# HKUST-Aerial-Robotics/Omni-swarm

Measured on AMD Instinct MI355X. Metric: keyframes/sec (4x fisheye 600x480) + p50 loop-match ms @ 100k-frame DB, higher is better.
Workload: dtype f16

## Files before the change

### include/omni_hip.h

```cpp
#ifndef OMNI_HIP_H
#define OMNI_HIP_H

#include <stddef.h>
#include <stdint.h>

#ifdef __cplusplus
extern "C" {
#endif

#define OMNI_ABI_VERSION 2

enum {
    OMNI_OK = 0,
    OMNI_ERR_INVALID = 1,
    OMNI_ERR_HIP = 2,
    OMNI_ERR_NOMEM = 3,
    OMNI_ERR_CAPACITY = 4
};

enum { OMNI_PREC_F32 = 0,
       OMNI_PREC_F16 = 1,
       OMNI_PREC_SPLIT = 2 };

enum { OMNI_STORE_F32 = 0, OMNI_STORE_F16 = 1 };
// ... 53 lines not shown

static inline void omni_fisheye_mask_rows(int height, int fisheye_mask, int* row0, int* row1) {
    *row0 = fisheye_mask ? height * 3 / 4 : height;
    *row1 = fisheye_mask ? height * 3 / 4 + height / 4 : height;
}

int omni_sp_infer(omni_sp* sp, const uint8_t* gray_host, int stride, int batch, int fisheye_mask,
                  float* kps_xy, int* n_kps, float* desc, float* scores);
int omni_sp_enqueue_dev(omni_sp* sp, const uint8_t* gray_dev, int stride, int batch, int fisheye_mask);
int omni_sp_fetch(omni_sp* sp, int batch, float* kps_xy, int* n_kps, float* desc, float* scores);
int omni_sp_dev_outputs(omni_sp* sp, const float** kps_xy_dev, const int** n_kps_dev, const float** desc_dev,
                        const float** scores_dev);
int omni_sp_get_dense(omni_sp* sp, int batch, float* semi_host, float* desc_host);
int omni_sp_postprocess_dense(omni_sp* sp, const float* semi_host, const float* desc_host, int batch,
                              float* kps_xy, int* n_kps, float* desc, float* scores);
int omni_sp_debug_layer(omni_sp* sp, const char* name, int batch, float* out_nchw_host, int* C, int* H, int* W);
#define OMNI_SP_NUM_STAGES 16
int         omni_sp_profile(omni_sp* sp, const uint8_t* gray_dev, int stride, int batch, int reps, float* stage_ms);
int         omni_sp_set_perf(omni_sp* sp, int on);
int         omni_sp_last_stage_ms(omni_sp* sp, float* stage_ms);
const char* omni_sp_stage_name(int stage);
double      omni_sp_stage_flops(const omni_sp* sp, int stage);
double      omni_sp_stage_tiles_left_out(const omni_sp* sp, int stage);
int         omni_sp_mask_skip_plan(int width, int height, int precision, int layer, int* rect, double* frac);

enum { OMNI_VLAD_CONV3X3_RELU6 = 0, OMNI_VLAD_PW_RELU6 = 1, OMNI_VLAD_DW3X3_RELU6 = 2,
       OMNI_VLAD_PW_LINEAR = 3, OMNI_VLAD_PW_LINEAR_RES = 4 };
typedef struct omni_vlad_layer {
    int kind, cin, cout, stride;
    const float* weight;
    const float* bias;
} omni_vlad_layer;
typedef struct omni_vlad_weights {
    int n_layers;
    const omni_vlad_layer* layers;
    int n_clusters, feat_dim, out_dim;
    const float* assign_w;
    const float* assign_b;
    const float* clusters;
    const float* fc_w;
    const float* fc_b;
} omni_vlad_weights;

omni_vlad* omni_vlad_create(omni_ctx* ctx, const omni_vlad_weights* w, int width, int height, int max_batch);
void       omni_vlad_destroy(omni_vlad* v);
int        omni_vlad_set_precision(omni_vlad* v, int precision);
// ... 169 lines not shown
```

### omni-swarm_amd/capi.py

```python
from __future__ import annotations

import ctypes as C
import os

import numpy as np

_HERE = os.path.dirname(os.path.abspath(__file__))
LIB_PATH = os.environ.get("OMNI_LIB") or os.path.join(_HERE, "lib", "libomni_hip.so")

OK, ERR_INVALID, ERR_HIP, ERR_NOMEM, ERR_CAPACITY = 0, 1, 2, 3, 4
PREC_F32, PREC_F16, PREC_SPLIT = 0, 1, 2
STORE_F32, STORE_F16 = 0, 1
BF_OPENCV, BF_MUTUAL = 0, 1
ABI_VERSION = 2
SP_NUM_LAYERS = 12
SP_NUM_STAGES = 16
SP_LAYER_NAMES = ["conv1a", "conv1b", "conv2a", "conv2b", "conv3a", "conv3b", "conv4a", "conv4b",
                  "convPa", "convPb", "convDa", "convDb"]
VB_NAMES = ["hblock", "sblock", "mblock", "pw_mfma3", "valu"]
VLAD_STEM_NAMES = ["stem", "stem_b0", "layers"]
VLAD_KINDS = {"conv3x3": 0, "pw_relu6": 1, "dw3x3_relu6": 2, "pw_linear": 3, "pw_linear_res": 4}

SYMBOLS = [
    "omni_abi_version", "omni_last_error", "omni_ctx_create", "omni_ctx_create_priority", "omni_ctx_order_after", "omni_memcpy_d2h_async", "omni_ctx_destroy", "omni_ctx_sync", "omni_ctx_stream",
    "omni_ctx_device_info", "omni_ctx_mfma_ceiling", "omni_dev_alloc", "omni_dev_free", "omni_host_alloc", "omni_host_free", "omni_memcpy_h2d", "omni_memcpy_d2h", "omni_timer_start",
    "omni_timer_stop", "omni_sp_create", "omni_sp_destroy", "omni_sp_desc_dim", "omni_sp_image_size", "omni_sp_infer", "omni_sp_enqueue_dev",
    "omni_sp_fetch", "omni_sp_dev_outputs", "omni_sp_get_dense", "omni_sp_postprocess_dense", "omni_sp_debug_layer",
    "omni_sp_profile", "omni_sp_stage_name", "omni_sp_stage_flops", "omni_sp_stage_tiles_left_out", "omni_sp_mask_skip_plan", "omni_vlad_create", "omni_vlad_destroy", "omni_vlad_set_precision", "omni_vlad_pack_block", "omni_sp_pack_constants",
    "omni_vlad_infer", "omni_vlad_enqueue_dev", "omni_vlad_fetch", "omni_vlad_dev_output", "omni_vlad_mask_skip_layers", "omni_vlad_debug_taps", "omni_vlad_debug_layer", "omni_vlad_block_paths", "omni_index_create",
    "omni_index_destroy", "omni_index_add", "omni_index_add_dev", "omni_index_ntotal", "omni_index_dim", "omni_index_reset", "omni_index_truncate", "omni_index_cert_stats",
    "omni_index_search", "omni_index_search_dev", "omni_index_search_prefix_dev", "omni_index_search_batch_prefix_dev", "omni_index_set_shard", "omni_topk_merge", "omni_index_last_scan_ms",
    "omni_index_save", "omni_index_load",
    "omni_trace_push", "omni_trace_pop", "omni_sp_set_perf", "omni_sp_last_stage_ms", "omni_bf_match", "omni_bf_match_multi", "omni_bf_match_batched_dev", "omni_config_count", "omni_config_describe", "omni_config_value", "omni_config_is_process_wide", "omni_cam_create", "omni_cam_create_mono", "omni_cam_destroy", "omni_cam_enqueue_dev", "omni_cam_enqueue_host", "omni_cam_enqueue_host_parts", "omni_cam_enqueue_fisheye_dev", "omni_cam_enqueue_fisheye_host", "omni_cam_get_input", "omni_cam_wait", "omni_cam_order_after", "omni_cam_set_active", "omni_cam_ready",
    "omni_shard_unique_id", "omni_shard_library_path", "omni_shard_create", "omni_shard_destroy", "omni_shard_ntotal", "omni_shard_preload_local", "omni_shard_step_batch_dev", "omni_shard_step_enqueue", "omni_shard_rows_consumed", "omni_shard_step_wait", "omni_shard_last_exchange_us",
    "omni_shard_search", "omni_flatten_create", "omni_flatten_destroy", "omni_flatten_out_bytes", "omni_flatten_enqueue_dev",
    "omni_resize_create", "omni_resize_destroy", "omni_resize_mode", "omni_resize_enqueue_dev", "omni_cam_enqueue_raw_dev", "omni_cam_enqueue_raw_host", "omni_cam_enqueue_raw_host_parts",
    "omni_landmarks_enqueue_dev", "omni_cam_set_stereo_model", "omni_cam_set_poses", "omni_cam_landmarks",
    "omni_homography_ransac_multi", "omni_bf_match_homography_multi", "omni_pnp_ransac_multi",
    "omni_jpeg_create", "omni_jpeg_destroy", "omni_jpeg_enqueue_dev", "omni_jpeg_header", "omni_jpeg_encode_host", "omni_cam_set_jpeg", "omni_cam_jpeg",
]
JPEG_OK, JPEG_TRUNCATED, JPEG_HEADER_BYTES = 0, 1, 328
HG_UNFILTERED, HG_OK, HG_NO_MODEL, HG_HOST = 0, 1, 2, 3
PNP_SKIPPED, PNP_OK, PNP_NO_MODEL, PNP_HOST = 0, 1, 2, 3
PNP_MAX_POINTS, PNP_MAX_ITERS = 2048, 1000


class OmniError(RuntimeError):
    pass


class _SpWeights(C.Structure):
# ... 84 lines not shown
    sig("omni_dev_free", C.c_int, [_vp, _vp])
    sig("omni_host_alloc", _vp, [C.c_size_t])
    sig("omni_host_free", C.c_int, [_vp])
    sig("omni_memcpy_h2d", C.c_int, [_vp, _vp, _vp, C.c_size_t])
    sig("omni_memcpy_d2h", C.c_int, [_vp, _vp, _vp, C.c_size_t])
    sig("omni_timer_start", C.c_int, [_vp])
    sig("omni_timer_stop", C.c_int, [_vp, _fp])
    sig("omni_sp_create", _vp, [_vp, C.POINTER(_SpWeights), _fp, _fp, C.c_int, C.c_int, C.c_int, C.c_float, C.c_int,
                                C.c_int, C.c_int])
    sig("omni_sp_destroy", None, [_vp])
    sig("omni_sp_desc_dim", C.c_int, [_vp])
    sig("omni_sp_infer", C.c_int, [_vp, _vp, C.c_int, C.c_int, C.c_int, _fp, _ip, _fp, _fp])
    sig("omni_sp_enqueue_dev", C.c_int, [_vp, _vp, C.c_int, C.c_int, C.c_int])
    sig("omni_sp_fetch", C.c_int, [_vp, C.c_int, _fp, _ip, _fp, _fp])
    sig("omni_sp_dev_outputs", C.c_int, [_vp, C.POINTER(_vp), C.POINTER(_vp), C.POINTER(_vp), C.POINTER(_vp)])
    sig("omni_sp_get_dense", C.c_int, [_vp, C.c_int, _fp, _fp])
    sig("omni_sp_postprocess_dense", C.c_int, [_vp, _fp, _fp, C.c_int, _fp, _ip, _fp, _fp])
    sig("omni_sp_debug_layer", C.c_int, [_vp, C.c_char_p, C.c_int, _fp, _ip, _ip, _ip])
    sig("omni_sp_profile", C.c_int, [_vp, _vp, C.c_int, C.c_int, C.c_int, _fp])
    sig("omni_sp_stage_name", C.c_char_p, [C.c_int])
    sig("omni_sp_stage_flops", C.c_double, [_vp, C.c_int])
    sig("omni_sp_stage_tiles_left_out", C.c_double, [_vp, C.c_int])
    sig("omni_sp_mask_skip_plan", C.c_int, [C.c_int, C.c_int, C.c_int, C.c_int, C.POINTER(C.c_int), C.POINTER(C.c_double)])
    sig("omni_vlad_create", _vp, [_vp, C.POINTER(_VladWeights), C.c_int, C.c_int, C.c_int])
    sig("omni_vlad_destroy", None, [_vp])
    sig("omni_vlad_set_precision", C.c_int, [_vp, C.c_int])
    sig("omni_sp_pack_constants", C.c_int64, [C.c_int, _fp, _fp, C.c_int, _vp, C.c_int64, C.POINTER(C.c_float)])
    sig("omni_vlad_pack_block", C.c_int64, [C.c_int, C.c_int, C.c_int, C.c_int, _fp, _fp, _fp, _fp, _fp, _vp, C.c_int64])
    sig("omni_vlad_infer", C.c_int, [_vp, _vp, C.c_int, C.c_int, C.c_int, _fp])
    sig("omni_vlad_enqueue_dev", C.c_int, [_vp, _vp, C.c_int, C.c_int, C.c_int])
    sig("omni_vlad_fetch", C.c_int, [_vp, C.c_int, _fp])
    sig("omni_vlad_dev_output", C.c_int, [_vp, C.POINTER(_vp)])
    sig("omni_vlad_mask_skip_layers", C.c_int, [_vp, C.POINTER(C.c_double), C.c_int])
    sig("omni_vlad_debug_taps", C.c_int, [_vp, C.c_int])
    sig("omni_vlad_debug_layer", C.c_int, [_vp, C.c_char_p, C.c_int, _fp, _ip, _ip, _ip])
    sig("omni_vlad_block_paths", C.c_int, [_vp, _ip, C.c_int])
    sig("omni_index_create", _vp, [_vp, C.c_int, C.c_int, C.c_int64])
    sig("omni_index_destroy", None, [_vp])
    sig("omni_index_add", C.c_int, [_vp, C.c_int64, _fp])
    sig("omni_index_add_dev", C.c_int, [_vp, C.c_int64, _vp])
    sig("omni_index_ntotal", C.c_int64, [_vp])
    sig("omni_index_reset", C.c_int, [_vp])
    sig("omni_index_truncate", C.c_int, [_vp, C.c_int64])
    sig("omni_index_cert_stats", C.c_int, [_vp, _i64p, _i64p])
    sig("omni_index_dim", C.c_int, [_vp])
    sig("omni_sp_image_size", C.c_int, [_vp, C.POINTER(C.c_int), C.POINTER(C.c_int)])
# ... 633 lines not shown
        src = self.ctx.to_device(g)
        out = self.ctx.to_device(np.full(n * self.capacity + guard, 0xA5, np.uint8))
        meta = self.ctx.to_device(np.full(2 * n, -1, np.int32))
        try:
            self.enqueue_dev(src, st, n, self.h_img if zero_from_row < 0 else zero_from_row, out, meta, meta + 4 * n)
            raw = self.ctx.from_device(out, (n * self.capacity + guard,), np.uint8)
            m = self.ctx.from_device(meta, (2, n), np.int32)
        finally:
            for p in (src, out, meta):
                self.ctx.free(p)
        self.last_raw = raw[:n * self.capacity].reshape(n, self.capacity)
        self.last_guard_ok = bool((raw[n * self.capacity:] == 0xA5).all())
        self.last_sizes = m[0].copy()
        return [(int(m[1, i]), self.last_raw[i, :m[0, i]].tobytes()) for i in range(n)]
SHARD_ID_BYTES = 128


def shard_unique_id() -> bytes:
    buf = C.create_string_buffer(SHARD_ID_BYTES)
    _check(lib().omni_shard_unique_id(buf))
    return buf.raw


def sp_mask_skip_plan(width: int, height: int, precision: int, layer: int):
    rect = (C.c_int * 4)()
    frac = C.c_double()
    _check(lib().omni_sp_mask_skip_plan(width, height, precision, layer, rect, C.byref(frac)))
    return tuple(rect), frac.value


def config_table() -> list:
    out = []
    for i in range(lib().omni_config_count()):
        env, doc = C.c_char_p(), C.c_char_p()
        d, lo, hi, cls = C.c_int(), C.c_int(), C.c_int(), C.c_int()
        _check(lib().omni_config_describe(i, C.byref(env), C.byref(d), C.byref(lo), C.byref(hi), C.byref(cls), C.byref(doc)))
        out.append({"env": env.value.decode(), "default": d.value, "lo": lo.value, "hi": hi.value, "cls": cls.value, "doc": doc.value.decode()})
    return out


def config_value(env: str) -> int:
    v = C.c_int()
    _check(lib().omni_config_value(env.encode(), C.byref(v)))
    return v.value


# ... 291 lines not shown
```

### omni-swarm_amd/csrc/config.h

```cpp
#pragma once
#include "common.h"

namespace omni {

enum CfgId {
    CFG_CONV_V1 = 0, CFG_RS_TRN, CFG_DET16, CFG_SP_SPARSE_DESC, CFG_SP_SPARSE_DA, CFG_SP_FUSED_CAND, CFG_SP_SPLIT_DB, CFG_SP_MASK_SKIP, CFG_SP_MASK_SKIP_SPLIT, CFG_SPLIT_FUSE1A, CFG_SPLIT_WINO,
    CFG_SPLIT_TRN, CFG_CONV_XCD, CFG_SP_PROFILE_MASK, CFG_PP_U8, CFG_PP_TRACE, CFG_PP_DBG, CFG_RS_TRACE, CFG_SPLIT_TRACE, CFG_SPLIT_DBG, CFG_WINO_TRACE, CFG_ROCTX,
    CFG_VLAD_BIG, CFG_VLAD_STEM_FUSE, CFG_VLAD_UNFUSED, CFG_VLAD_MFMA, CFG_VLAD_SBLOCK, CFG_VLAD_MBLOCK_PX, CFG_VLAD_MFMA_PX, CFG_VLAD_FC_MFMA, CFG_VLAD_MBLOCK_CPW,
    CFG_VLAD_SB_LDSPAD, CFG_VLAD_SB_PERSIST, CFG_VLAD_SB_TRACE, CFG_VLAD_SB_DBG, CFG_VLAD_MASK_SKIP,
    CFG_SCAN_ROWS_MIN, CFG_MQ_ROT, CFG_MQ_MIN, CFG_INDEX_MIRROR, CFG_INDEX_MIRROR_MIN_ROWS, CFG_INDEX_CERT_FAIL,
    CFG_GEOMETRY_THREADS, CFG_MESSAGE_THREADS, CFG_GEOMETRY_ASYNC, CFG_DETECTOR_ASYNC, CFG_PIPELINE_ONE_STREAM, CFG_PIPELINE_FIFO, CFG_PIPELINE_UNIT_PLAN,
    CFG_HW_QUEUES,
    CFG_RCCL_LIB,
    CFG_COUNT
};
enum CfgClass {
    CFG_VARIANT = 0,
    CFG_TUNING = 1,
    CFG_DEBUG = 2,
    CFG_TEST = 3,
    CFG_STRING = 4
};
struct CfgOption { const char* env; int def, lo, hi; int cls; const char* doc; };
extern const CfgOption kCfgOptions[CFG_COUNT];

struct Config {
    int v[CFG_COUNT];
    int operator[](CfgId i) const { return v[i]; }
};
// ... 6 lines not shown
```

### omni-swarm_amd/csrc/config.hip

```cpp
#include "config.h"

#include <atomic>
#include <cerrno>
#include <climits>
#include <cstdlib>

namespace omni {

const CfgOption kCfgOptions[CFG_COUNT] = {
    {"OMNI_CONV_V1", 0, 0, 3, CFG_VARIANT, "fp16 3x3 layers: 0 = production (conv1a fused into the ping-pong conv1b, register-stationary cin=128); 1 = generic kernel, 2 = persistent LDS-DMA kernel, "
                                           "3 = ping-pong without the conv1a fusion -- 1-3 exist only in the test build of the library (lib_test/)"},
    {"OMNI_RS_TRN", -1, -1, 1, CFG_VARIANT, "register-stationary kernel of the unpooled cin=128 fp16 layers: tile orientation, -1 = the one with fewer tiles, 0 = plain, 1 = transposed"},
    {"OMNI_DET16", 1, 0, 1, CFG_VARIANT, "detector head of the fp16 and OMNI_PREC_SPLIT paths on v_mfma_f32_32x32x16_f16 with split (hi, lo) operands (0: the exact-f32 MFMA kernel)"},
    {"OMNI_SP_SPARSE_DESC", 1, 0, 1, CFG_VARIANT, "convDb + descriptor norm only at the cells around the key points (0: dense descriptor map)"},
    {"OMNI_SP_SPARSE_DA", 1, 0, 1, CFG_VARIANT, "convDa only at those cells too (fp16 and OMNI_PREC_SPLIT; 0: dense convDa)"},
    {"OMNI_SP_FUSED_CAND", 1, 0, 1, CFG_VARIANT, "getKeyPoints' threshold inside the detector head's epilogue + window masks from the candidate list (0: sp_cand_kernel re-reads the heat map)"},
    {"OMNI_SP_SPLIT_DB", 1, 0, 1, CFG_VARIANT, "OMNI_PREC_SPLIT: convDb + descriptor norm at the key points' cells with split (hi, lo) operands on the fp16 matrix cores (0: exact-f32 MFMA convolution)"},
    {"OMNI_SP_MASK_SKIP", 1, 0, 1, CFG_VARIANT, "fp16: the tiles inside the constant region of the fisheye mask are left out of the tile walk (0: every tile)"},
    {"OMNI_SP_MASK_SKIP_SPLIT", 1, 0, 1, CFG_VARIANT, "the same for OMNI_PREC_SPLIT"},
    {"OMNI_SPLIT_FUSE1A", 1, 0, 1, CFG_VARIANT, "OMNI_PREC_SPLIT: conv1a built inside the conv1b kernel from the u8 image (0: separate exact-f32 conv1a pass)"},
    {"OMNI_SPLIT_WINO", 7, 0, 15, CFG_VARIANT, "OMNI_PREC_SPLIT: the cin = 64 layers as Winograd F(2x2,3x3) kernels with split operands (conv_wino.hip), bit 0 = conv1b (with the conv1a "
                                                "fusion), 1 = conv2a, 2 = conv2b, 3 = conv3a (off by default: same time as the direct kernel, profiles/r06g); 0: the direct kernels of conv_split.hip"},
    {"OMNI_SPLIT_TRN", -1, -1, 1, CFG_VARIANT, "OMNI_PREC_SPLIT cin=128 kernel: tile orientation, as OMNI_RS_TRN"},
    {"OMNI_CONV_XCD", 1, 0, 1, CFG_VARIANT, "persistent convolution kernels derive (cout group, tile walk) from an XCD-aware block id: the cout groups of a pixel tile and its neighbours "
                                           "share one L2 (0: plain blockIdx; process-wide, same results either way)"},
    {"OMNI_SP_PROFILE_MASK", 0, 0, 1, CFG_TUNING, "omni_sp_profile times the stages with the fisheye mask on (what the key-frame pipeline runs)"},
    {"OMNI_PP_U8", 1, 0, 1, CFG_VARIANT, "fp16 conv1a inside conv1b's kernel: matrix-core operands straight from the image bytes (0: through the 256-entry u8 -> (hi, lo) table in LDS)"},
    {"OMNI_PP_TRACE", 0, 0, 1, CFG_DEBUG, "s_memtime trace of the ping-pong conv kernel on stderr"},
    {"OMNI_PP_DBG", 0, 0, 255, CFG_DEBUG, "ping-pong conv kernel timing ablations (WRONG results)"},
    {"OMNI_RS_TRACE", 0, 0, 1, CFG_DEBUG, "s_memtime trace of the register-stationary kernel"},
    {"OMNI_SPLIT_TRACE", 0, 0, 1, CFG_DEBUG, "s_memtime trace of the split-precision kernel"},
    {"OMNI_SPLIT_DBG", 0, 0, 3, CFG_DEBUG, "split-precision kernel timing ablations: 1 = no stores, 2 = every DMA reads tile 0 (WRONG results)"},
    {"OMNI_WINO_TRACE", 0, 0, 1, CFG_DEBUG, "s_memtime trace of the Winograd split kernel"},
    {"OMNI_ROCTX", 0, 0, 1, CFG_DEBUG, "roctx ranges around upload / SuperPoint / MobileNetVLAD / post-processing / BF match / index add + search / exchange and the host loop's "
                                      "stages (rocprofv3 --marker-trace; the library is resolved by dlopen)"},
    {"OMNI_VLAD_BIG", 0, 0, 128, CFG_TUNING, "64 / 128: the 64- / 128-pixel tiles of the unfused block kernel (measured slower at 600x480)"},
    {"OMNI_VLAD_STEM_FUSE", 1, 0, 1, CFG_VARIANT, "stem + block 0 in one kernel (0: two kernels)"},
    {"OMNI_VLAD_UNFUSED", 0, 0, 1, CFG_VARIANT, "1: every block as expand / depthwise / project launches"},
    {"OMNI_VLAD_MFMA", 1, 0, 1, CFG_VARIANT, "late blocks' 1x1 convolutions on the matrix cores"},
    {"OMNI_VLAD_SBLOCK", 1, 0, 1, CFG_VARIANT, "fused split-fp16 block kernel (vlad_s.hip)"},
    {"OMNI_VLAD_MBLOCK_PX", 2048, 0, 1 << 24, CFG_TUNING, "fused matrix-core block kernel for blocks of at most this many input pixels per image (0 disables)"},
    {"OMNI_VLAD_MFMA_PX", 0, 0, 1 << 24, CFG_TUNING, "> 0: matrix-core 1x1 convolutions for blocks of at most this many input pixels per image (default 2048)"},
// ... 122 lines not shown
```

### omni-swarm_amd/csrc/conv.h

```cpp
#pragma once
#include "common.h"
#include "tile_walk.h"

namespace omni {

#define CONV_TH 8
#define CONV_TW 32
#define RS_TH 6
#define RS_TW 32
int conv_rs_pool_tile_rows();
#define CONV_COUT_TILE 64
#define CONV_CIN_CHUNK 64

static inline size_t conv_packed_elems(int cin, int cout, int ksize) { return (size_t)cin * cout * ksize * ksize; }

void conv_pack_weights_f16(const float* w_oihw, int cin, int cout, int ksize, __half* out);
void conv_pack_weights_f32(const float* w_oihw, int cin, int cout, int ksize, float* out);

struct ConvArgs {
    const void* in;
    void* out;
    const void* w_packed;
    const float* bias;
    int batch, H, W, cin, cout, ksize;
    int in_cstride = 0;
    bool relu, pool;
    bool out_f32;
    int n_cu = 0;
    const void* zero_page = nullptr;
    float split_inv = 0.f;
    int variant = 0;
    int skip_ty0 = 0, skip_ty1 = 0, skip_tx0 = 0, skip_tx1 = 0;
};
int conv_mfma(hipStream_t stream, int precision, const ConvArgs& a);
int conv_read_pixel_f16(hipStream_t stream, const void* map, int Ho, int Wo, int C, int y, int x, void* vec);
int conv_fill_rect_f16(hipStream_t stream, void* map, int batch, int Ho, int Wo, int C, int y0, int y1, int x0, int x1, const void* vec);
int conv_read_pixel_bytes(hipStream_t stream, const void* map, int64_t row_bytes, int64_t org_bytes, int pix_bytes, int y, int x, void* vec);
int conv_fill_rect_bytes(hipStream_t stream, void* map, int batch, int64_t img_bytes, int64_t row_bytes, int64_t org_bytes, int pix_bytes, int y0, int y1, int x0, int x1,
                         const void* vec);

float conv_pack_weights_split(const float* w_oihw, int cin, int cout, uint16_t* out);
float conv_split_act_scale();
int conv_split(hipStream_t stream, const ConvArgs& a);
int conv1a_split(hipStream_t stream, const uint8_t* gray, int stride, int batch, int H, int W, int fisheye_mask, const float* w, const float* bias,
                 const float* u8_lut, void* out_split, int skip_tr0 = 0, int skip_tr1 = 0);
int split_to_nchw_f32(hipStream_t stream, const void* in_split, float* out, int batch, int C, int H, int W);
void conv1a_split_pack_fused(const float* w , const float* bias , uint16_t* frag );
int conv1ab_split_fused(hipStream_t stream, const ConvArgs& a, const uint8_t* gray, int gstride, int fisheye_mask, const void* w1a_frag, const uint32_t* lut_hl);
float conv_pack_weights_wino(const float* w_oihw, int cin, int cout, uint16_t* out);
int conv_wino(hipStream_t stream, const ConvArgs& a, bool out_split);
int conv1ab_wino_fused(hipStream_t stream, const ConvArgs& a, const uint8_t* gray, int gstride, int fisheye_mask, const void* w1a_frag, const uint32_t* lut_hl, bool out_split);
int split_to_raw32(hipStream_t stream, const void* in_split, void* out_raw, int batch, int C, int H, int W);
int conv_read_pixels2x2_bytes(hipStream_t stream, const void* map, int64_t row_bytes, int64_t org_bytes, int pix_bytes, int y, int x, void* vec);
int conv_fill_rect2x2_bytes(hipStream_t stream, void* map, int batch, int64_t img_bytes, int64_t row_bytes, int64_t org_bytes, int pix_bytes, int y0, int y1, int x0, int x1,
                            const void* vec);
int raw32_to_nchw_f32(hipStream_t stream, const void* in_raw, float* out, int batch, int C, int H, int W);
__host__ __device__ inline int split_frame_w(int W) { return ((W + 31) & ~31) + 2; }
__host__ __device__ inline int split_frame_h(int H) { return ((H + 31) & ~31) + 2; }
inline size_t split_frame_bytes(int H, int W, int C) { return (size_t)split_frame_h(H) * split_frame_w(W) * C * 4; }

int conv1ab_fused(hipStream_t stream, const ConvArgs& a, const uint8_t* gray, int gstride, int fisheye_mask, const _Float16* w1a_frag,
                  const float* bias1a, const uint32_t* lut_hl);
// ... 46 lines not shown
```

### omni-swarm_amd/csrc/conv.hip

```cpp
#include "config.h"
#include "conv.h"
#include <type_traits>

namespace omni {

typedef _Float16 half8_t __attribute__((ext_vector_type(8)));
typedef _Float16 half4_t __attribute__((ext_vector_type(4)));
typedef float floatx16 __attribute__((ext_vector_type(16)));
typedef float floatx4 __attribute__((ext_vector_type(4)));

template <typename T, int KG, int EPL>
static void pack_weights(const float* w, int cin, int cout, int ks, T* out) {
    const int taps = ks * ks, n_ct = cout / 64, n_ch = cin / 64;
    size_t o = 0;
    for (int ct = 0; ct < n_ct; ++ct)
        for (int ch = 0; ch < n_ch; ++ch)
            for (int tap = 0; tap < taps; ++tap)
                for (int kg = 0; kg < KG; ++kg)
                    for (int m = 0; m < 2; ++m)
                        for (int l = 0; l < 64; ++l)
                            for (int e = 0; e < EPL; ++e) {
                                const int co = ct * 64 + m * 32 + (l & 31);
                                const int ci = ch * 64 + kg * (64 / KG) + (l >> 5) * EPL + e;
                                const float v = w[((size_t)co * cin + ci) * taps + tap];
// ... 2343 lines not shown
    const int y = (int)(by % rh);
    const int64_t b = by / rh;
    *reinterpret_cast<uint4*>(map + b * img_bytes + org_bytes + (y0 + y) * row_bytes + ((int64_t)(x0 + x) * chunks + c) * 16) = vec[c];
}
int conv_read_pixel_bytes(hipStream_t st, const void* map, int64_t row_bytes, int64_t org_bytes, int pix_bytes, int y, int x, void* vec) {
    OMNI_REQUIRE(pix_bytes % 16 == 0 && y >= 0 && x >= 0 && (org_bytes + y * row_bytes + (int64_t)x * pix_bytes) % 16 == 0, OMNI_ERR_INVALID, "conv_read_pixel_bytes: bad pixel");
    const int chunks = pix_bytes / 16;
    hipLaunchKernelGGL(read_pixel_f16_kernel, dim3(cdiv(chunks, 64)), dim3(64), 0, st, (const uint4*)map, (org_bytes + y * row_bytes + (int64_t)x * pix_bytes) / 16, chunks, (uint4*)vec);
    OMNI_LAUNCH_CHECK();
    return OMNI_OK;
}
int conv_fill_rect_bytes(hipStream_t st, void* map, int batch, int64_t img_bytes, int64_t row_bytes, int64_t org_bytes, int pix_bytes, int y0, int y1, int x0, int x1,
                         const void* vec) {
    OMNI_REQUIRE(pix_bytes % 16 == 0 && img_bytes % 16 == 0 && row_bytes % 16 == 0 && org_bytes % 16 == 0 && y0 >= 0 && x0 >= 0, OMNI_ERR_INVALID, "conv_fill_rect_bytes: bad layout");
    if (y1 <= y0 || x1 <= x0 || batch <= 0) return OMNI_OK;
    const int chunks = pix_bytes / 16;
    const int64_t total = (int64_t)batch * (y1 - y0) * (x1 - x0) * chunks;
    hipLaunchKernelGGL(fill_rect_bytes_kernel, dim3((unsigned)cdiv64(total, 256)), dim3(256), 0, st, (char*)map, img_bytes, row_bytes, org_bytes, chunks, y0, x0, y1 - y0,
                       x1 - x0, (const uint4*)vec, total);
    OMNI_LAUNCH_CHECK();
    return OMNI_OK;
}

}
```

### omni-swarm_amd/csrc/superpoint.hip

```cpp
#include <algorithm>
#include <vector>

#include "config.h"
#include "conv.h"
#include "sp_plan.h"
#include "sp_post.h"

namespace {
struct LayerDef { const char* name; int cin, cout, ks, div; bool pool; };
const LayerDef kLayers[OMNI_SP_NUM_LAYERS] = {
    {"conv1a", 1, 64, 3, 1, false},    {"conv1b", 64, 64, 3, 1, true},     {"conv2a", 64, 64, 3, 2, false},    {"conv2b", 64, 64, 3, 2, true},
    {"conv3a", 64, 128, 3, 4, false},  {"conv3b", 128, 128, 3, 4, true},   {"conv4a", 128, 128, 3, 8, false},  {"conv4b", 128, 128, 3, 8, false},
    {"convPa", 128, 256, 3, 8, false}, {"convPb", 256, 65, 1, 8, false},   {"convDa", 128, 256, 3, 8, false},  {"convDb", 256, 256, 1, 8, false}};
enum { L1A = 0, L1B, L2A, L2B, L3A, L3B, L4A, L4B, LPA, LPB, LDA, LDB };
enum { ST_CONV1A = 0, ST_CONV1B, ST_CONV2A, ST_CONV2B, ST_CONV3A, ST_CONV3B, ST_CONV4A, ST_CONV4B, ST_HEADS_A,
       ST_DET_TAIL, ST_DESC_TAIL, ST_POST, ST_COUNT };
const char* kStageNames[OMNI_SP_NUM_STAGES] = {
    "conv1a", "conv1b+pool", "conv2a", "conv2b+pool", "conv3a", "conv3b+pool", "conv4a", "conv4b", "convPa|convDa",
    "convPb+softmax+d2s", "convDb+l2norm", "nms+topk+describe", "", "", "", ""};
}

struct omni_sp {
    omni_ctx* ctx = nullptr;
    omni::Config cfg;
// ... 20 lines not shown
    void* wDbFragHi = nullptr; void* wDbFragLo = nullptr;
    float* bias_heads = nullptr;
    float* lut = nullptr;
    uint16_t* w1a_frag = nullptr;
    uint32_t* lut_hl = nullptr;
    void* wpk_w[OMNI_SP_NUM_LAYERS] = {};
    float winv_w[OMNI_SP_NUM_LAYERS] = {};
    void* a_tmp = nullptr;
    float* pca_compT = nullptr;
    float* pca_mean = nullptr;
    void *a1a = nullptr, *a1b = nullptr, *a2a = nullptr, *a2b = nullptr, *a3a = nullptr, *a3b = nullptr, *a4a = nullptr,
         *a4b = nullptr, *heads = nullptr;
    float *draw = nullptr, *semi = nullptr;
    uint8_t* gray_stage = nullptr;
    omni::SpPostBuffers pb = {};
    omni::HostBuf hstage;
    omni::DevBuf dense_tmp;
    hipEvent_t ev[OMNI_SP_NUM_STAGES + 1] = {};
    hipEvent_t ev_convs = nullptr;
    bool perf = false, perf_valid = false;
    struct MaskSkip {
        int ty0 = 0, ty1 = 0, tx0 = 0, tx1 = 0;
        int oy0 = 0, oy1 = 0, ox0 = 0, ox1 = 0;
        int oh = 0, ow = 0, oc = 0;
        int pix_bytes = 0;
        int64_t row_bytes = 0, img_bytes = 0, org_bytes = 0;
        void* vec = nullptr;
        void** map = nullptr;
        double frac = 0.0;
    };
    MaskSkip mskip[6];
    uint8_t* zero_gray = nullptr;
    size_t zero_gray_bytes = 0;
    std::mutex mu;
};

namespace omni {

template <typename T>
static int dev_upload(omni_sp* s, T** dst, const void* src, size_t bytes) {
    hipStream_t st = s->ctx->stream;
    if (int rc = s->mem.alloc(dst, bytes)) return rc;
    OMNI_HIP_TRY(hipMemcpyAsync(*dst, src, bytes, hipMemcpyHostToDevice, st));
    OMNI_HIP_TRY(hipStreamSynchronize(st));
    return OMNI_OK;
}

static void sp_mask_skip_rects(int H, int W, bool split, omni_sp::MaskSkip (&ks)[6]) {
    int m0, m1;
    omni_fisheye_mask_rows(H, 1, &m0, &m1);
    int h = H, w = W;
    for (auto& k : ks) k = omni_sp::MaskSkip{};
    int a = m0 + 1, b = (m1 == h) ? h - 1 : m1 - 2, c = 0, d = w - 1;
    if (split && b >= a) {
        omni_sp::MaskSkip& k = ks[0];
        k.ty0 = (a + 7) / 8; k.ty1 = (b + 1) / 8; k.tx0 = 0; k.tx1 = (w + 31) / 32;
        if (k.ty1 <= k.ty0) k.ty0 = k.ty1 = k.tx0 = k.tx1 = 0;
        k.oy0 = k.ty0 * 8; k.oy1 = k.ty1 * 8 < h ? k.ty1 * 8 : h; k.ox0 = 0; k.ox1 = k.ty1 > k.ty0 ? w : 0;
        k.oh = h; k.ow = w; k.oc = 64;
        k.frac = (double)(k.ty1 - k.ty0) / ((h + 7) / 8);
    }
    const bool pool[5] = {true, false, true, false, true};
    const int chans[5] = {64, 64, 64, 128, 128};
    static_assert(CONV_TW == 32, "tile width");
    const int TW = 32;
    for (int i = 0; i < 5; ++i) {
        const int TH = split ? (i == 4 ? 2 : 4) : (i == 4 ? conv_rs_pool_tile_rows() : CONV_TH);
        a += 1; b -= 1; c += 1; d -= 1;
        omni_sp::MaskSkip& k = ks[1 + i];
        if (b < a || d < c) break;
        k.ty0 = (a + TH - 1) / TH; k.ty1 = (b + 1) / TH; k.tx0 = (c + TW - 1) / TW; k.tx1 = (d + 1) / TW;
        if (k.ty1 <= k.ty0 || k.tx1 <= k.tx0) k.ty0 = k.ty1 = k.tx0 = k.tx1 = 0;
        k.frac = (double)(k.ty1 - k.ty0) * (k.tx1 - k.tx0) / ((double)((h + TH - 1) / TH) * ((w + TW - 1) / TW));
        const int f = pool[i] ? 2 : 1;
        k.oy0 = k.ty0 * TH / f; k.oy1 = k.ty1 * TH / f; k.ox0 = k.tx0 * TW / f; k.ox1 = k.tx1 * TW / f;
        if (pool[i]) { a = (a + 1) / 2; b = (b - 1) >> 1; c = (c + 1) / 2; d = (d - 1) >> 1; h /= 2; w /= 2; }
        k.oh = h; k.ow = w; k.oc = chans[i];
    }
}

static int sp_plan_mask_skip(omni_sp* s) {
    s->facts.mask_skip = false;
    const bool split = s->precision == OMNI_PREC_SPLIT;
    if (s->facts.conv_variant != 0 || s->precision == OMNI_PREC_F32) return OMNI_OK;
    if (!s->cfg[split ? CFG_SP_MASK_SKIP_SPLIT : CFG_SP_MASK_SKIP]) return OMNI_OK;
    sp_mask_skip_rects(s->H, s->W, split, s->mskip);
    void** maps[6] = {&s->a1a, &s->a1b, &s->a2a, &s->a2b, &s->a3a, &s->a3b};
    for (int i = 0; i < 6; ++i) {
        omni_sp::MaskSkip& k = s->mskip[i];
        k.map = maps[i];
        if (k.oc == 0) continue;
        if (split) {
            k.pix_bytes = k.oc * 4;
            k.row_bytes = (int64_t)split_frame_w(k.ow) * k.pix_bytes;
            k.img_bytes = (int64_t)split_frame_bytes(k.oh, k.ow, k.oc);
            k.org_bytes = k.row_bytes + k.pix_bytes;
        } else {
            k.pix_bytes = k.oc * 2; k.row_bytes = (int64_t)k.ow * k.pix_bytes; k.img_bytes = k.row_bytes * k.oh; k.org_bytes = 0;
        }
        if (k.ty1 > k.ty0) {
            if (int rc = s->mem.alloc(&k.vec, (size_t)k.pix_bytes * 4)) return rc;
            s->facts.mask_skip = true;
        }
    }
    return OMNI_OK;
}

static void sp_set_facts(omni_sp* s) {
    SpHandleFacts& f = s->facts;
    f.precision = s->precision; f.H = s->H; f.W = s->W;
    f.conv_variant = s->cfg[CFG_CONV_V1];
    f.det16 = s->cfg[CFG_DET16] != 0;
    f.fused_cand = s->cfg[CFG_SP_FUSED_CAND] != 0;
    f.sparse_desc = s->cfg[CFG_SP_SPARSE_DESC] != 0;
    f.sparse_da = s->cfg[CFG_SP_SPARSE_DA] != 0;
    f.split_fuse1a = s->cfg[CFG_SPLIT_FUSE1A] != 0;
    f.split_db = s->cfg[CFG_SP_SPLIT_DB] != 0;
    f.wino = sp_wino_layers(s->precision, s->cfg[CFG_SPLIT_WINO], s->H, s->W, f.split_fuse1a);
}

static int sp_init(omni_sp* s, const omni_sp_weights* w, const float* pca_comp, const float* pca_mean) {
    hipStream_t st = s->ctx->stream;
    int rc;
// ... 136 lines not shown
    s->pb.pca_mean = s->pca_mean;
    for (int i = 0; i <= OMNI_SP_NUM_STAGES; ++i) OMNI_HIP_TRY(hipEventCreate(&s->ev[i]));
    OMNI_HIP_TRY(hipEventCreateWithFlags(&s->ev_convs, hipEventDisableTiming));
    OMNI_HIP_TRY(hipStreamSynchronize(st));
    return sp_plan_mask_skip(s);
}

static int tails_prec(const SpPassPlan& p) { return p.tails_f32 ? OMNI_PREC_F32 : OMNI_PREC_F16; }

enum SpKernelFamily { SP_K_DIRECT, SP_K_WINO };
static ConvArgs sp_layer_args(const omni_sp* s, const SpPassPlan& p, int l, SpKernelFamily fam, const void* in, void* out, int batch, int cout = 0) {
    const LayerDef& d = kLayers[l];
    const bool split = s->precision == OMNI_PREC_SPLIT, wino = fam == SP_K_WINO;
    ConvArgs a;
    a.in = in; a.out = out; a.batch = batch; a.H = s->H / d.div; a.W = s->W / d.div; a.cin = d.cin; a.cout = cout ? cout : d.cout; a.ksize = d.ks;
    a.relu = l != LDB; a.pool = d.pool;
    a.out_f32 = l == LDB || (l == LPA && split);
    if (l == LDB) a.in_cstride = 512;
    a.w_packed = wino ? s->wpk_w[l] : s->wpk[l];
    a.split_inv = wino ? s->winv_w[l] : s->winv[l];
    a.bias = l == LPA ? s->bias_heads : (split && !a.out_f32) ? s->bias_s[l] : s->bias[l];
    a.n_cu = s->ctx->prop.multiProcessorCount; a.zero_page = s->ctx->zero_page; a.variant = s->facts.conv_variant;
    const int i = l == L1B ? 1 : l == L2A ? 2 : l == L2B ? 3 : l == L3A ? 4 : l == L3B ? 5 : -1;
    if (p.use_skip && i >= 0) { a.skip_ty0 = s->mskip[i].ty0; a.skip_ty1 = s->mskip[i].ty1; a.skip_tx0 = s->mskip[i].tx0; a.skip_tx1 = s->mskip[i].tx1; }
    return a;
}
static int sp_conv(omni_sp* s, const SpPassPlan& p, int l, const void* in, void* out, int batch, int cout = 0) {
    const ConvArgs a = sp_layer_args(s, p, l, SP_K_DIRECT, in, out, batch, cout);
    if (l == LDB) return conv_mfma(s->ctx->stream, tails_prec(p), a);
    return s->precision == OMNI_PREC_SPLIT ? conv_split(s->ctx->stream, a) : conv_mfma(s->ctx->stream, s->precision, a);
}
static int sp_heads_layer(omni_sp* s, const SpPassPlan& p, int batch, bool cpa_only) {
    return sp_conv(s, p, LPA, s->a4b, cpa_only ? s->headsP : s->heads, batch, cpa_only ? 256 : 512);
}
static const void* sp_cda(const omni_sp* s) { return (const char*)s->heads + (size_t)256 * s->esz; }
static int sp_desc_dense_f16(omni_sp* s, int batch) {
    return convdb_l2norm(s->ctx->stream, s->ctx, sp_cda(s), 512, s->wDbFrag, s->bias[LDB], s->draw, (int64_t)batch * s->Hc * s->Wc);
}
static int sp_desc_dense_generic(omni_sp* s, const SpPassPlan& p, int batch) {
    if (int rc = sp_conv(s, p, LDB, sp_cda(s), s->draw, batch)) return rc;
    return l2norm_channels(s->ctx->stream, s->draw, (int64_t)batch * s->Hc * s->Wc);
}
static SpSparseDesc sp_sparse_desc(const omni_sp* s, const SpPassPlan& p) {
    SpSparseDesc sd;
    sd.mode = p.desc; sd.split_db = p.desc_split_db; sd.cand_fused = p.cand_fused;
    sd.ctx = s->ctx; sd.cda = sp_cda(s); sd.in_cstride = 512; sd.bias = s->bias[LDB];
    sd.wfrag = s->wDbFrag; sd.wdb_hi = s->wDbFragHi; sd.wdb_lo = s->wDbFragLo; sd.wdb_f32 = s->wpk[LDB];
    sd.a4b = s->a4b; sd.da_w = s->wpk[LPA]; sd.da_bias = s->bias_heads; sd.da_g32_first = 8; sd.da_inv = s->winv[LPA]; sd.da_compact = s->da_compact;
    sd.cx = s->cx32; sd.cy = s->cy32; sd.n_cu = s->ctx->prop.multiProcessorCount; sd.zero_page = s->ctx->zero_page;
    return sd;
}

static int sp_forward(omni_sp* s, const uint8_t* gray_dev, int stride, int batch, int fisheye_mask, bool with_events, bool run_post, bool calibrating = false);
static int sp_calibrate_mask_skip(omni_sp* s, int stride, int zero_image_offset) {
    hipStream_t st = s->ctx->stream;
    int rc;
    const size_t need = (size_t)stride * s->H + 4;
    if (s->zero_gray_bytes < need) {
        s->mem.release_one(s->zero_gray);
        s->zero_gray = nullptr; s->zero_gray_bytes = 0;
        if ((rc = s->mem.alloc(&s->zero_gray, need, st, true))) return rc;
        s->zero_gray_bytes = need;
    }
    if ((rc = sp_forward(s, s->zero_gray + zero_image_offset, stride, 1, 1, false, false, true))) return rc;
    const SpPassPlan& cal = s->last;
    for (const omni_sp::MaskSkip& k : s->mskip) {
        if (k.ty1 <= k.ty0 || (k.map == &s->a1a && cal.conv1a == SP_1A_FUSED)) continue;
        if ((k.map == &s->a2a && cal.conv2a.wino) || (k.map == &s->a3a && cal.conv3a.wino)) {
            if ((rc = conv_read_pixels2x2_bytes(st, *k.map, k.row_bytes, k.org_bytes, k.pix_bytes, ((k.oy0 + k.oy1) / 2) & ~1, ((k.ox0 + k.ox1) / 2) & ~1, k.vec))) return rc;
            if ((rc = conv_fill_rect2x2_bytes(st, *k.map, s->max_batch, k.img_bytes, k.row_bytes, k.org_bytes, k.pix_bytes, k.oy0, k.oy1, k.ox0, k.ox1, k.vec))) return rc;
            continue;
        }
        if ((rc = conv_read_pixel_bytes(st, *k.map, k.row_bytes, k.org_bytes, k.pix_bytes, (k.oy0 + k.oy1) / 2, (k.ox0 + k.ox1) / 2, k.vec))) return rc;
        if ((rc = conv_fill_rect_bytes(st, *k.map, s->max_batch, k.img_bytes, k.row_bytes, k.org_bytes, k.pix_bytes, k.oy0, k.oy1, k.ox0, k.ox1, k.vec))) return rc;
    }
    return OMNI_OK;
}

static SpPostParams post_params(const omni_sp* s) {
    SpPostParams p;
    p.width = s->W; p.height = s->H; p.thres = s->thres; p.max_num = s->max_num; p.dist_thresh = 4; p.pca_dim = s->pca_dim;
    return p;
}

static int sp_forward(omni_sp* s, const uint8_t* gray_dev, int stride, int batch, int fisheye_mask, bool with_events, bool run_post, bool calibrating) {
    hipStream_t st = s->ctx->stream;
    const int H = s->H, W = s->W, n_cu = s->ctx->prop.multiProcessorCount;
    int rc, stage = 0;
    if ((rc = s->ctx->ensure_zero_page())) return rc;
// ... 294 lines not shown
    switch (stage) {
        case ST_CONV1A: return c(H, W, 1, 64, 3);
        case ST_CONV1B: return c(H, W, 64, 64, 3);
        case ST_CONV2A: case ST_CONV2B: return c(H / 2, W / 2, 64, 64, 3);
        case ST_CONV3A: return c(H / 4, W / 4, 64, 128, 3);
        case ST_CONV3B: return c(H / 4, W / 4, 128, 128, 3);
        case ST_CONV4A: case ST_CONV4B: return c(H / 8, W / 8, 128, 128, 3);
        case ST_HEADS_A: return c(H / 8, W / 8, 128, 512, 3);
        case ST_DET_TAIL: return c(H / 8, W / 8, 256, 65, 1);
        case ST_DESC_TAIL: return c(H / 8, W / 8, 256, 256, 1);
        default: return 0.0;
    }
}

int omni_sp_mask_skip_plan(int width, int height, int precision, int layer, int* rect, double* frac) {
    OMNI_REQUIRE(width > 0 && height > 0 && layer >= 0 && layer < 6, OMNI_ERR_INVALID, "bad argument");
    omni_sp::MaskSkip ks[6];
    if (precision != OMNI_PREC_F32) omni::sp_mask_skip_rects(height, width, precision == OMNI_PREC_SPLIT, ks);
    if (rect) { rect[0] = ks[layer].ty0; rect[1] = ks[layer].ty1; rect[2] = ks[layer].tx0; rect[3] = ks[layer].tx1; }
    if (frac) *frac = ks[layer].ty1 > ks[layer].ty0 ? ks[layer].frac : 0.0;
    return OMNI_OK;
}

double omni_sp_stage_tiles_left_out(const omni_sp* s, int stage) {
    if (!s || !s->facts.mask_skip) return 0.0;
    const int i = stage == ST_CONV1A ? 0 : stage == ST_CONV1B ? 1 : stage == ST_CONV2A ? 2 : stage == ST_CONV2B ? 3 : stage == ST_CONV3A ? 4 : stage == ST_CONV3B ? 5 : -1;
    return i < 0 ? 0.0 : s->mskip[i].frac;
}

int64_t omni_sp_pack_constants(int which, const float* w, const float* bias, int cout, uint16_t* out, int64_t out_halfs, float* scale) {
    if (!w || !out || !scale) { omni::set_error("omni_sp_pack_constants: null argument"); return -2; }
    if (which == 0) {
        if (!bias || out_halfs < 2048) { omni::set_error("omni_sp_pack_constants: conv1a needs a bias and 2048 halfs"); return -2; }
        omni::conv1a_pack_u8_weights(w, bias, out);
        *scale = 1.f;
        return 2048;
    }
    if (which == 1) {
        const int64_t need = (int64_t)64 * cout * 32;
        if (cout < 64 || cout % 64 || out_halfs < need) { omni::set_error("omni_sp_pack_constants: cout %d, %lld halfs", cout, (long long)out_halfs); return -2; }
        *scale = omni::conv_pack_weights_wino(w, 64, cout, out);
        return need;
    }
    omni::set_error("omni_sp_pack_constants: which = %d", which);
    return -2;
}

int omni_sp_set_perf(omni_sp* s, int on) {
    OMNI_REQUIRE(s, OMNI_ERR_INVALID, "null handle");
    std::lock_guard<std::mutex> lk(s->mu);
// ... 43 lines not shown
```

Baseline: 2599.

## Skip the image-independent bottom band of fisheye mask tiles in SuperPoint convs

The masked tile skip changes from an interior rectangle of constant-output tiles to a full-width band of tile rows that runs from where the mask starts to the bottom of the image. The output there does not depend on the image. At calibration the band's activations from a zero image are computed once into slot 0 and copied to the other batch slots by a new kernel. This lets the convolution tile walk drop whole rows, so more tiles may be skipped than with the rectangle. The old rectangle path is kept behind a test config flag. The risk is correctness if the band is not truly image-independent, for example through receptive-field edges.

```diff
diff --git a/include/omni_hip.h b/include/omni_hip.h
--- a/include/omni_hip.h
+++ b/include/omni_hip.h
@@ -99,6 +99,7 @@
 const char* omni_sp_stage_name(int stage);
 double      omni_sp_stage_flops(const omni_sp* sp, int stage);
 double      omni_sp_stage_tiles_left_out(const omni_sp* sp, int stage);
+int         omni_sp_mask_band_plan(int width, int height, int precision, int layer, int* ty0, int* tiles_y, double* frac);
 int         omni_sp_mask_skip_plan(int width, int height, int precision, int layer, int* rect, double* frac);
 
 enum { OMNI_VLAD_CONV3X3_RELU6 = 0, OMNI_VLAD_PW_RELU6 = 1, OMNI_VLAD_DW3X3_RELU6 = 2,
diff --git a/omni-swarm_amd/capi.py b/omni-swarm_amd/capi.py
--- a/omni-swarm_amd/capi.py
+++ b/omni-swarm_amd/capi.py
@@ -26,7 +26,7 @@
     "omni_ctx_device_info", "omni_ctx_mfma_ceiling", "omni_dev_alloc", "omni_dev_free", "omni_host_alloc", "omni_host_free", "omni_memcpy_h2d", "omni_memcpy_d2h", "omni_timer_start",
     "omni_timer_stop", "omni_sp_create", "omni_sp_destroy", "omni_sp_desc_dim", "omni_sp_image_size", "omni_sp_infer", "omni_sp_enqueue_dev",
     "omni_sp_fetch", "omni_sp_dev_outputs", "omni_sp_get_dense", "omni_sp_postprocess_dense", "omni_sp_debug_layer",
-    "omni_sp_profile", "omni_sp_stage_name", "omni_sp_stage_flops", "omni_sp_stage_tiles_left_out", "omni_sp_mask_skip_plan", "omni_vlad_create", "omni_vlad_destroy", "omni_vlad_set_precision", "omni_vlad_pack_block", "omni_sp_pack_constants",
+    "omni_sp_profile", "omni_sp_stage_name", "omni_sp_stage_flops", "omni_sp_stage_tiles_left_out", "omni_sp_mask_skip_plan", "omni_sp_mask_band_plan", "omni_vlad_create", "omni_vlad_destroy", "omni_vlad_set_precision", "omni_vlad_pack_block", "omni_sp_pack_constants",
     "omni_vlad_infer", "omni_vlad_enqueue_dev", "omni_vlad_fetch", "omni_vlad_dev_output", "omni_vlad_mask_skip_layers", "omni_vlad_debug_taps", "omni_vlad_debug_layer", "omni_vlad_block_paths", "omni_index_create",
     "omni_index_destroy", "omni_index_add", "omni_index_add_dev", "omni_index_ntotal", "omni_index_dim", "omni_index_reset", "omni_index_truncate", "omni_index_cert_stats",
     "omni_index_search", "omni_index_search_dev", "omni_index_search_prefix_dev", "omni_index_search_batch_prefix_dev", "omni_index_set_shard", "omni_topk_merge", "omni_index_last_scan_ms",
@@ -157,6 +157,7 @@
     sig("omni_sp_stage_flops", C.c_double, [_vp, C.c_int])
     sig("omni_sp_stage_tiles_left_out", C.c_double, [_vp, C.c_int])
     sig("omni_sp_mask_skip_plan", C.c_int, [C.c_int, C.c_int, C.c_int, C.c_int, C.POINTER(C.c_int), C.POINTER(C.c_double)])
+    sig("omni_sp_mask_band_plan", C.c_int, [C.c_int, C.c_int, C.c_int, C.c_int, C.POINTER(C.c_int), C.POINTER(C.c_int), C.POINTER(C.c_double)])
     sig("omni_vlad_create", _vp, [_vp, C.POINTER(_VladWeights), C.c_int, C.c_int, C.c_int])
     sig("omni_vlad_destroy", None, [_vp])
     sig("omni_vlad_set_precision", C.c_int, [_vp, C.c_int])
@@ -836,6 +837,12 @@
     return buf.raw
 
 
+def sp_mask_band_plan(width: int, height: int, precision: int, layer: int):
+    ty0, tiles_y, frac = C.c_int(), C.c_int(), C.c_double()
+    _check(lib().omni_sp_mask_band_plan(width, height, precision, layer, C.byref(ty0), C.byref(tiles_y), C.byref(frac)))
+    return ty0.value, tiles_y.value, frac.value
+
+
 def sp_mask_skip_plan(width: int, height: int, precision: int, layer: int):
     rect = (C.c_int * 4)()
     frac = C.c_double()
diff --git a/omni-swarm_amd/csrc/config.h b/omni-swarm_amd/csrc/config.h
--- a/omni-swarm_amd/csrc/config.h
+++ b/omni-swarm_amd/csrc/config.h
@@ -4,7 +4,7 @@
 namespace omni {
 
 enum CfgId {
-    CFG_CONV_V1 = 0, CFG_RS_TRN, CFG_DET16, CFG_SP_SPARSE_DESC, CFG_SP_SPARSE_DA, CFG_SP_FUSED_CAND, CFG_SP_SPLIT_DB, CFG_SP_MASK_SKIP, CFG_SP_MASK_SKIP_SPLIT, CFG_SPLIT_FUSE1A, CFG_SPLIT_WINO,
+    CFG_CONV_V1 = 0, CFG_RS_TRN, CFG_DET16, CFG_SP_SPARSE_DESC, CFG_SP_SPARSE_DA, CFG_SP_FUSED_CAND, CFG_SP_SPLIT_DB, CFG_SP_MASK_SKIP, CFG_SP_MASK_SKIP_SPLIT, CFG_SP_MASK_RECT, CFG_SPLIT_FUSE1A, CFG_SPLIT_WINO,
     CFG_SPLIT_TRN, CFG_CONV_XCD, CFG_SP_PROFILE_MASK, CFG_PP_U8, CFG_PP_TRACE, CFG_PP_DBG, CFG_RS_TRACE, CFG_SPLIT_TRACE, CFG_SPLIT_DBG, CFG_WINO_TRACE, CFG_ROCTX,
     CFG_VLAD_BIG, CFG_VLAD_STEM_FUSE, CFG_VLAD_UNFUSED, CFG_VLAD_MFMA, CFG_VLAD_SBLOCK, CFG_VLAD_MBLOCK_PX, CFG_VLAD_MFMA_PX, CFG_VLAD_FC_MFMA, CFG_VLAD_MBLOCK_CPW,
     CFG_VLAD_SB_LDSPAD, CFG_VLAD_SB_PERSIST, CFG_VLAD_SB_TRACE, CFG_VLAD_SB_DBG, CFG_VLAD_MASK_SKIP,
diff --git a/omni-swarm_amd/csrc/config.hip b/omni-swarm_amd/csrc/config.hip
--- a/omni-swarm_amd/csrc/config.hip
+++ b/omni-swarm_amd/csrc/config.hip
@@ -16,8 +16,10 @@
     {"OMNI_SP_SPARSE_DA", 1, 0, 1, CFG_VARIANT, "convDa only at those cells too (fp16 and OMNI_PREC_SPLIT; 0: dense convDa)"},
     {"OMNI_SP_FUSED_CAND", 1, 0, 1, CFG_VARIANT, "getKeyPoints' threshold inside the detector head's epilogue + window masks from the candidate list (0: sp_cand_kernel re-reads the heat map)"},
     {"OMNI_SP_SPLIT_DB", 1, 0, 1, CFG_VARIANT, "OMNI_PREC_SPLIT: convDb + descriptor norm at the key points' cells with split (hi, lo) operands on the fp16 matrix cores (0: exact-f32 MFMA convolution)"},
-    {"OMNI_SP_MASK_SKIP", 1, 0, 1, CFG_VARIANT, "fp16: the tiles inside the constant region of the fisheye mask are left out of the tile walk (0: every tile)"},
+    {"OMNI_SP_MASK_SKIP", 1, 0, 1, CFG_VARIANT, "fp16: the tile rows inside the image-independent band of the fisheye mask are left out of the tile walk (0: every tile)"},
     {"OMNI_SP_MASK_SKIP_SPLIT", 1, 0, 1, CFG_VARIANT, "the same for OMNI_PREC_SPLIT"},
+    {"OMNI_SP_MASK_RECT", 0, 0, 1, CFG_TEST, "1: a masked pass leaves out only the rectangle of tiles where the output is one constant vector, filled by broadcasting that vector "
+                                             "(what was skipped before the band: the A/B reference, same results)"},
     {"OMNI_SPLIT_FUSE1A", 1, 0, 1, CFG_VARIANT, "OMNI_PREC_SPLIT: conv1a built inside the conv1b kernel from the u8 image (0: separate exact-f32 conv1a pass)"},
     {"OMNI_SPLIT_WINO", 7, 0, 15, CFG_VARIANT, "OMNI_PREC_SPLIT: the cin = 64 layers as Winograd F(2x2,3x3) kernels with split operands (conv_wino.hip), bit 0 = conv1b (with the conv1a "
                                                 "fusion), 1 = conv2a, 2 = conv2b, 3 = conv3a (off by default: same time as the direct kernel, profiles/r06g); 0: the direct kernels of conv_split.hip"},
diff --git a/omni-swarm_amd/csrc/conv.h b/omni-swarm_amd/csrc/conv.h
--- a/omni-swarm_amd/csrc/conv.h
+++ b/omni-swarm_amd/csrc/conv.h
@@ -38,6 +38,7 @@
 int conv_read_pixel_bytes(hipStream_t stream, const void* map, int64_t row_bytes, int64_t org_bytes, int pix_bytes, int y, int x, void* vec);
 int conv_fill_rect_bytes(hipStream_t stream, void* map, int batch, int64_t img_bytes, int64_t row_bytes, int64_t org_bytes, int pix_bytes, int y0, int y1, int x0, int x1,
                          const void* vec);
+int conv_copy_slot0_bytes(hipStream_t stream, void* map, int slots, int64_t img_bytes, int64_t first_byte, int64_t bytes);
 
 float conv_pack_weights_split(const float* w_oihw, int cin, int cout, uint16_t* out);
 float conv_split_act_scale();
diff --git a/omni-swarm_amd/csrc/conv.hip b/omni-swarm_amd/csrc/conv.hip
--- a/omni-swarm_amd/csrc/conv.hip
+++ b/omni-swarm_amd/csrc/conv.hip
@@ -2389,4 +2389,21 @@
     return OMNI_OK;
 }
 
-}
+__global__ void copy_slot0_kernel(uint4* map, int64_t img_chunks, int64_t first_chunk, int64_t len_chunks, int64_t total) {
+    const int64_t i = (int64_t)blockIdx.x * blockDim.x + threadIdx.x;
+    if (i >= total) return;
+    const int64_t b = i / len_chunks + 1, c = i - (b - 1) * len_chunks;
+    map[b * img_chunks + first_chunk + c] = map[first_chunk + c];
+}
+int conv_copy_slot0_bytes(hipStream_t st, void* map, int slots, int64_t img_bytes, int64_t first_byte, int64_t bytes) {
+    OMNI_REQUIRE(map && slots >= 1 && img_bytes % 16 == 0 && first_byte % 16 == 0 && bytes % 16 == 0 && first_byte >= 0 && bytes > 0 && first_byte + bytes <= img_bytes,
+                 OMNI_ERR_INVALID, "conv_copy_slot0_bytes: block outside the image slot");
+    if (slots == 1) return OMNI_OK;
+    const int64_t len = bytes / 16, total = (int64_t)(slots - 1) * len;
+    OMNI_REQUIRE(cdiv64(total, 256) < (1ll << 31), OMNI_ERR_INVALID, "conv_copy_slot0_bytes: too large for one grid");
+    hipLaunchKernelGGL(copy_slot0_kernel, dim3((unsigned)cdiv64(total, 256)), dim3(256), 0, st, (uint4*)map, img_bytes / 16, first_byte / 16, len, total);
+    OMNI_LAUNCH_CHECK();
+    return OMNI_OK;
+}
+
+}
diff --git a/omni-swarm_amd/csrc/superpoint.hip b/omni-swarm_amd/csrc/superpoint.hip
--- a/omni-swarm_amd/csrc/superpoint.hip
+++ b/omni-swarm_amd/csrc/superpoint.hip
@@ -66,14 +66,17 @@
     struct MaskSkip {
         int ty0 = 0, ty1 = 0, tx0 = 0, tx1 = 0;
         int oy0 = 0, oy1 = 0, ox0 = 0, ox1 = 0;
+        int band_ty0 = 0, tiles_y = 0, tiles_x = 0;
+        int band_oy0 = 0;
         int oh = 0, ow = 0, oc = 0;
         int pix_bytes = 0;
         int64_t row_bytes = 0, img_bytes = 0, org_bytes = 0;
         void* vec = nullptr;
         void** map = nullptr;
-        double frac = 0.0;
+        double frac = 0.0, band_frac = 0.0;
     };
     MaskSkip mskip[6];
+    bool mask_band = false;
     uint8_t* zero_gray = nullptr;
     size_t zero_gray_bytes = 0;
     std::mutex mu;
@@ -108,16 +111,24 @@
     const int chans[5] = {64, 64, 64, 128, 128};
     static_assert(CONV_TW == 32, "tile width");
     const int TW = 32;
+    const bool to_bottom = m1 == H;
+    bool rect = true;
     for (int i = 0; i < 5; ++i) {
         const int TH = split ? (i == 4 ? 2 : 4) : (i == 4 ? conv_rs_pool_tile_rows() : CONV_TH);
         a += 1; b -= 1; c += 1; d -= 1;
         omni_sp::MaskSkip& k = ks[1 + i];
-        if (b < a || d < c) break;
-        k.ty0 = (a + TH - 1) / TH; k.ty1 = (b + 1) / TH; k.tx0 = (c + TW - 1) / TW; k.tx1 = (d + 1) / TW;
-        if (k.ty1 <= k.ty0 || k.tx1 <= k.tx0) k.ty0 = k.ty1 = k.tx0 = k.tx1 = 0;
-        k.frac = (double)(k.ty1 - k.ty0) * (k.tx1 - k.tx0) / ((double)((h + TH - 1) / TH) * ((w + TW - 1) / TW));
         const int f = pool[i] ? 2 : 1;
-        k.oy0 = k.ty0 * TH / f; k.oy1 = k.ty1 * TH / f; k.ox0 = k.tx0 * TW / f; k.ox1 = k.tx1 * TW / f;
+        k.tiles_y = (h + TH - 1) / TH; k.tiles_x = (w + TW - 1) / TW;
+        k.band_ty0 = to_bottom ? std::min((a + TH - 1) / TH, k.tiles_y) : k.tiles_y;
+        k.band_oy0 = k.band_ty0 * TH / f;
+        k.band_frac = (double)(k.tiles_y - k.band_ty0) / k.tiles_y;
+        rect = rect && b >= a && d >= c;
+        if (rect) {
+            k.ty0 = (a + TH - 1) / TH; k.ty1 = (b + 1) / TH; k.tx0 = (c + TW - 1) / TW; k.tx1 = (d + 1) / TW;
+            if (k.ty1 <= k.ty0 || k.tx1 <= k.tx0) k.ty0 = k.ty1 = k.tx0 = k.tx1 = 0;
+            k.frac = (double)(k.ty1 - k.ty0) * (k.tx1 - k.tx0) / ((double)k.tiles_y * k.tiles_x);
+            k.oy0 = k.ty0 * TH / f; k.oy1 = k.ty1 * TH / f; k.ox0 = k.tx0 * TW / f; k.ox1 = k.tx1 * TW / f;
+        }
         if (pool[i]) { a = (a + 1) / 2; b = (b - 1) >> 1; c = (c + 1) / 2; d = (d - 1) >> 1; h /= 2; w /= 2; }
         k.oh = h; k.ow = w; k.oc = chans[i];
     }
@@ -129,6 +140,8 @@
     if (s->facts.conv_variant != 0 || s->precision == OMNI_PREC_F32) return OMNI_OK;
     if (!s->cfg[split ? CFG_SP_MASK_SKIP_SPLIT : CFG_SP_MASK_SKIP]) return OMNI_OK;
     sp_mask_skip_rects(s->H, s->W, split, s->mskip);
+    s->mask_band = false;
+    for (int i = 1; i < 6 && !s->cfg[CFG_SP_MASK_RECT]; ++i) s->mask_band = s->mask_band || s->mskip[i].band_ty0 < s->mskip[i].tiles_y;
     void** maps[6] = {&s->a1a, &s->a1b, &s->a2a, &s->a2b, &s->a3a, &s->a3b};
     for (int i = 0; i < 6; ++i) {
         omni_sp::MaskSkip& k = s->mskip[i];
@@ -142,7 +155,9 @@
         } else {
             k.pix_bytes = k.oc * 2; k.row_bytes = (int64_t)k.ow * k.pix_bytes; k.img_bytes = k.row_bytes * k.oh; k.org_bytes = 0;
         }
-        if (k.ty1 > k.ty0) {
+        if (s->mask_band && i > 0) {
+            if (k.band_ty0 < k.tiles_y) s->facts.mask_skip = true;
+        } else if (k.ty1 > k.ty0) {
             if (int rc = s->mem.alloc(&k.vec, (size_t)k.pix_bytes * 4)) return rc;
             s->facts.mask_skip = true;
         }
@@ -325,7 +340,11 @@
     a.bias = l == LPA ? s->bias_heads : (split && !a.out_f32) ? s->bias_s[l] : s->bias[l];
     a.n_cu = s->ctx->prop.multiProcessorCount; a.zero_page = s->ctx->zero_page; a.variant = s->facts.conv_variant;
     const int i = l == L1B ? 1 : l == L2A ? 2 : l == L2B ? 3 : l == L3A ? 4 : l == L3B ? 5 : -1;
-    if (p.use_skip && i >= 0) { a.skip_ty0 = s->mskip[i].ty0; a.skip_ty1 = s->mskip[i].ty1; a.skip_tx0 = s->mskip[i].tx0; a.skip_tx1 = s->mskip[i].tx1; }
+    if (p.use_skip && i >= 0) {
+        const omni_sp::MaskSkip& k = s->mskip[i];
+        if (s->mask_band) { a.skip_ty0 = k.band_ty0; a.skip_ty1 = k.tiles_y; a.skip_tx0 = 0; a.skip_tx1 = k.tiles_x; }
+        else { a.skip_ty0 = k.ty0; a.skip_ty1 = k.ty1; a.skip_tx0 = k.tx0; a.skip_tx1 = k.tx1; }
+    }
     return a;
 }
 static int sp_conv(omni_sp* s, const SpPassPlan& p, int l, const void* in, void* out, int batch, int cout = 0) {
@@ -368,6 +387,12 @@
     if ((rc = sp_forward(s, s->zero_gray + zero_image_offset, stride, 1, 1, false, false, true))) return rc;
     const SpPassPlan& cal = s->last;
     for (const omni_sp::MaskSkip& k : s->mskip) {
+        if (s->mask_band && k.map != &s->a1a) {
+            if (k.band_ty0 >= k.tiles_y || k.band_oy0 >= k.oh) continue;
+            const int64_t first = k.org_bytes + k.band_oy0 * k.row_bytes, bytes = (k.oh - 1 - k.band_oy0) * k.row_bytes + (int64_t)k.ow * k.pix_bytes;
+            if ((rc = conv_copy_slot0_bytes(st, *k.map, s->max_batch, k.img_bytes, first, bytes))) return rc;
+            continue;
+        }
         if (k.ty1 <= k.ty0 || (k.map == &s->a1a && cal.conv1a == SP_1A_FUSED)) continue;
         if ((k.map == &s->a2a && cal.conv2a.wino) || (k.map == &s->a3a && cal.conv3a.wino)) {
             if ((rc = conv_read_pixels2x2_bytes(st, *k.map, k.row_bytes, k.org_bytes, k.pix_bytes, ((k.oy0 + k.oy1) / 2) & ~1, ((k.ox0 + k.ox1) / 2) & ~1, k.vec))) return rc;
@@ -708,10 +733,20 @@
     return OMNI_OK;
 }
 
+int omni_sp_mask_band_plan(int width, int height, int precision, int layer, int* ty0, int* tiles_y, double* frac) {
+    OMNI_REQUIRE(width > 0 && height > 0 && layer >= 0 && layer < 6, OMNI_ERR_INVALID, "bad argument");
+    omni_sp::MaskSkip ks[6];
+    if (precision != OMNI_PREC_F32) omni::sp_mask_skip_rects(height, width, precision == OMNI_PREC_SPLIT, ks);
+    if (ty0) *ty0 = ks[layer].band_ty0;
+    if (tiles_y) *tiles_y = ks[layer].tiles_y;
+    if (frac) *frac = ks[layer].band_ty0 < ks[layer].tiles_y ? ks[layer].band_frac : 0.0;
+    return OMNI_OK;
+}
+
 double omni_sp_stage_tiles_left_out(const omni_sp* s, int stage) {
     if (!s || !s->facts.mask_skip) return 0.0;
     const int i = stage == ST_CONV1A ? 0 : stage == ST_CONV1B ? 1 : stage == ST_CONV2A ? 2 : stage == ST_CONV2B ? 3 : stage == ST_CONV3A ? 4 : stage == ST_CONV3B ? 5 : -1;
-    return i < 0 ? 0.0 : s->mskip[i].frac;
+    return i < 0 ? 0.0 : (s->mask_band && i > 0) ? s->mskip[i].band_frac : s->mskip[i].frac;
 }
 
 int64_t omni_sp_pack_constants(int which, const float* w, const float* bias, int cout, uint16_t* out, int64_t out_halfs, float* scale) {
```

After: 2691 (median of 6 runs). 1.04x the previous value.
